# callmeray/PointMVSNet

Measured on AMD Instinct MI355X. Metric: depth-maps/sec (DTU 640x512, 3 src views, 2 flow iters), higher is better.
Workload: dtype f32

## Files before the change

### include/pointflow_hip.h

```cpp
#ifndef POINTFLOW_HIP_H_
#define POINTFLOW_HIP_H_

#include <stdint.h>

#ifdef __cplusplus
extern "C" {
#endif

#define PF_OK 0
#define PF_ERR_INVALID_ARG (-1)
#define PF_ERR_UNSUPPORTED (-2)

#define PF_STATUS_BAD_INDEX 1u

#define PF_MAX_VIEWS 8
#define PF_GEMM_TILE 64

#define PF_CAM_KREF_INV 0
#define PF_CAM_RREF_INV 9
#define PF_CAM_TREF 18
#define PF_CAM_MEAN 21
#define PF_CAM_STD 24
#define PF_CAM_VIEWS 27
#define PF_CAM_VIEW_STRIDE 21
// ... 112 lines not shown

int pf_edge_backward_coeffs_f32(const double* partials, int G, int T, int cbn, int C, int concat, int groups_per_stat,
                                int Ng, int k, float* c1, float* c2, float* dgamma, float* dbeta, int accumulate,
                                void* stream);

int64_t pf_knn_inverse_workspace(int G, int Ng, int k);
int pf_knn_inverse(const int64_t* idx, int k, int G, int Ng, uint32_t* order, uint32_t* start, void* workspace,
                   int64_t workspace_bytes, void* stream);

int pf_norm_blocks(int64_t S);
int pf_channel_stats_f32(const float* x, int64_t N, int64_t C, int64_t S, double* partials, void* stream);
int pf_channel_affine_f32(const float* x, float* y, const float* scale, const float* shift, int64_t N, int64_t C,
                          int64_t S, int samples_per_stat, int relu, void* stream);
int pf_channel_bn_apply_f32(const float* x, float* y, const double* partials, int T, int64_t N, int64_t C, int64_t S,
                            int samples_per_stat, double count, const float* gamma, const float* beta,
                            float* running_mean, float* running_var, float momentum, float eps, int relu,
                            const float* addend, void* stream);
int pf_channel_bn_apply2_f32(const float* x1, const double* partials1, int T1, const float* gamma1, const float* beta1,
                             float* running_mean1, float* running_var1, float momentum1, float eps1, const float* x2,
                             const double* partials2, int T2, const float* gamma2, const float* beta2,
                             float* running_mean2, float* running_var2, float momentum2, float eps2, float* y, int64_t N,
                             int64_t C, int64_t S, int samples_per_stat, double count, void* stream);
int pf_channel_bn_fused_f32(const float* x, float* y, int64_t N, int64_t C, int64_t S, int samples_per_stat,
                            const float* gamma, const float* beta, float* running_mean, float* running_var,
                            float momentum, float eps, int relu, float* scale, float* shift, int ld_affine,
                            void* stream);

int pf_conv3d_blocks(int64_t Cin, int64_t Cout, int64_t Di, int64_t Hi, int64_t Wi, int stride);
int pf_conv3d_k3_f32(const float* x, const float* wp, float* y, int64_t N, int64_t Cin, int64_t Cout, int64_t Di,
                     int64_t Hi, int64_t Wi, int stride, const float* in_scale, const float* in_shift,
                     const pf_bn_job* in_bn, int samples_per_stat, double* partials, void* stream);
int pf_conv3d_pair_blocks(int64_t Cin, int64_t Cout, int64_t D, int64_t H, int64_t W);
int pf_conv3d_k3_pair_f32(const float* x, const float* wp, float* y, int64_t N, int64_t Cin, int64_t Cout, int64_t D,
                          int64_t H, int64_t W, double* partials, void* stream);
int pf_conv3d_k3_few_f32(const float* x, const float* w, float* y, int64_t N, int64_t Cin, int64_t Cout, int64_t D,
                         int64_t H, int64_t W, void* stream);

int pf_deconv3d_blocks(int64_t D, int64_t H, int64_t W);
int pf_deconv3d_k3s2_f32(const float* xa, const float* xb, const float* w, float* y, int64_t N, int64_t Cin,
                         int64_t Cout, int64_t D, int64_t H, int64_t W, const float* in_scale, const float* in_shift,
                         const pf_bn_job* in_bn, int samples_per_stat, double* partials, void* stream);

int pf_conv3d_bottom_supported(int64_t Cin, int64_t Cout, int stride);
int pf_conv3d_bottom_blocks(int64_t Di, int64_t Hi, int64_t Wi, int stride);
int pf_conv3d_bottom_f32(const float* x, const float* wp, float* y, int64_t N, int64_t Cin, int64_t Cout, int64_t Di,
                         int64_t Hi, int64_t Wi, int stride, const float* in_scale, const float* in_shift,
                         const pf_bn_job* in_bn, int samples_per_stat, double* partials, void* stream);
int pf_deconv3d_bottom_supported(int64_t Cin, int64_t Cout);
int pf_deconv3d_bottom_blocks(int64_t Di, int64_t Hi, int64_t Wi);
int pf_deconv3d_bottom_f32(const float* x, const float* wp, float* y, int64_t N, int64_t Cin, int64_t Cout, int64_t Di,
                           int64_t Hi, int64_t Wi, const float* in_scale, const float* in_shift, const pf_bn_job* in_bn,
                           int samples_per_stat, double* partials, void* stream);

int pf_conv2d_wide_supported(int64_t Cin, int64_t Cout, int kernel_size, int stride);
int pf_conv2d_wide_blocks(int64_t Cout, int64_t Hi, int64_t Wi, int stride);
int pf_conv2d_wide_f32(const float* x, const float* wp, float* y, int64_t N, int64_t Cin, int64_t Cout, int64_t Hi,
                       int64_t Wi, int kernel_size, int stride, const float* in_scale, const float* in_shift,
                       const pf_bn_job* in_bn, int samples_per_stat, double* partials, int out_channel_last,
                       void* stream);
int pf_conv2d_wide_sets_f32(const float* x, int x_layout, const float* wp, int64_t wp_set_stride, int sets, float* y,
                            int64_t N, int64_t Cin, int64_t Cout, int64_t Hi, int64_t Wi, int kernel_size, int stride,
                            const float* in_scale, const float* in_shift, const pf_bn_job* in_bn, int samples_per_stat,
                            double* partials, int out_channel_last, void* stream);

int pf_flow_head_f32(const float* Z, int64_t ldz, const float* scale, const float* shift, int ld_affine,
                     const pf_bn_job* in_bn, const float* w_out, const float* depth_in, int dh, int dw,
                     const float* interval, int h, int w, int ratio, float* flow_prob, float* depth_out,
// ... 117 lines not shown
```

### pointmvsnet_amd/_lib.py

```python
import ctypes
import os

import torch

_HERE = os.path.dirname(os.path.abspath(__file__))
LIB_PATH = os.environ.get("PF_LIB_PATH") or os.path.join(_HERE, "libpointflow_hip.so")

_vp, _i, _i64, _f, _d = ctypes.c_void_p, ctypes.c_int, ctypes.c_int64, ctypes.c_float, ctypes.c_double



class BnJob(ctypes.Structure):
    _fields_ = [("partials", _vp), ("T", ctypes.c_int32), ("pcols", ctypes.c_int32), ("col0", ctypes.c_int32),
                ("C", ctypes.c_int32), ("count", _d), ("unbias_n", _d), ("gamma", _vp), ("beta", _vp),
                ("running_mean", _vp), ("running_var", _vp), ("momentum", _f), ("eps", _f),
                ("G", ctypes.c_int32), ("groups_per_stat", ctypes.c_int32), ("scale", _vp), ("shift", _vp),
                ("ld_affine", ctypes.c_int32), ("rows4", ctypes.c_int32)]


class WgradItem(ctypes.Structure):
    _fields_ = [("gr", _vp), ("x", _vp)] + [(n, _i64) for n in ("N", "Cg", "Cx", "Do", "Ho", "Wo", "Di", "Hi", "Wi")] + \
               [(n, ctypes.c_int32) for n in ("KD", "KH", "KW", "stride", "pd", "ph", "pw", "x_samples_per_stat")] + \
               [("x_scale", _vp), ("x_shift", _vp), ("workspace", _vp), ("workspace_bytes", _i64)] + \
               [(n, _i64) for n in ("rows_P", "ldg", "ldx", "x_rows_per_stat")]


PROTOTYPES = {
    "pf_version": ([], ctypes.c_char_p),
    "pf_error_string": ([_i], ctypes.c_char_p),
    "pf_device_info": ([ctypes.POINTER(_i), ctypes.POINTER(_i), ctypes.c_char_p, _i], _i),
    "pf_debug_timestamp": ([_vp, _vp], _i),
    "pf_check_status": ([ctypes.POINTER(ctypes.c_uint), _vp], _i),
    "pf_gather_knn_forward_f32": ([_vp, _vp, _vp, _i64, _i64, _i64, _i64, _vp], _i),
    "pf_gather_knn_forward_f64": ([_vp, _vp, _vp, _i64, _i64, _i64, _i64, _vp], _i),
    "pf_gather_knn_backward_f32": ([_vp, _vp, _vp, _i64, _i64, _i64, _i64, _vp, _vp, _vp], _i),
    "pf_gather_knn_backward_f64": ([_vp, _vp, _vp, _i64, _i64, _i64, _i64, _vp, _vp, _vp], _i),
    "pf_knn_lattice_f32": ([_vp, ctypes.POINTER(_i64), _i64, _i64, _i64, _i64, _i, _i, _vp, _vp, _vp], _i),
    "pf_fetch_forward_f32": ([_vp, _vp, _vp, _vp, _vp, _i64, _i64, _i64, _i64, _i64, _i64, _vp], _i),
    "pf_fetch_backward_f32": ([_vp, _vp, _vp, _vp, _vp, _i64, _i64, _i64, _i64, _i64, _i64, _vp], _i),
    "pf_fetch_variance_f32": ([_vp, _vp, _vp, _vp, _vp, _i64, _i64, _i64, _i64, _i64, _i64, _i, _vp], _i),
    "pf_frustum_variance_f32": ([_vp, _vp, _vp, _vp, _vp, _vp, _vp, _vp, _vp, _i64, _i64, _i64, _i64, _i64, _i64, _vp], _i),
    "pf_frustum_variance_cl_f32": ([_vp, _vp, _vp, _vp, _vp, _vp, _vp, _vp, _vp, _i64, _i64, _i64, _i64, _i64, _i64, _vp], _i),
    "pf_nchw_to_nhwc_f32": ([_vp, _vp, _i64, _i64, _i64, _vp], _i),
    "pf_resize_bilinear_f32": ([_vp, _vp, _i64, _i64, _i64, _i64, _i64, _vp], _i),
    "pf_flow_pyramid_f32": ([_vp, _i, _i, _i, _vp, _i, _i, _i, _vp, _i, _i, _i, _i, _i, _i, _vp, _vp, _vp,
                             ctypes.POINTER(_vp), ctypes.POINTER(_vp), _vp], _i),
    "pf_flow_features_f32": ([_vp, _vp, _vp, _i, _i, _i, _i, _i, _i, _vp, _i, _i, _vp, _vp, _i, _vp, _vp, _vp], _i),
    "pf_stat_blocks": ([_i, _i], _i),
    "pf_gemm_blocks": ([_i, _i], _i),
    "pf_pointwise_gemm_f32": ([_vp, _i, _i64, _vp, _vp, _i64, _i, _i, _i, _i, _i, _vp, _vp, ctypes.POINTER(BnJob), _i,
                               _vp, _vp], _i),
    "pf_conv3d_blocks": ([_i64, _i64, _i64, _i64, _i64, _i], _i),
    "pf_conv3d_k3_f32": ([_vp, _vp, _vp, _i64, _i64, _i64, _i64, _i64, _i64, _i, _vp, _vp, ctypes.POINTER(BnJob), _i,
                          _vp, _vp], _i),
    "pf_conv3d_pair_blocks": ([_i64, _i64, _i64, _i64, _i64], _i),
    "pf_conv3d_k3_pair_f32": ([_vp, _vp, _vp, _i64, _i64, _i64, _i64, _i64, _i64, _vp, _vp], _i),
    "pf_conv3d_k3_few_f32": ([_vp, _vp, _vp, _i64, _i64, _i64, _i64, _i64, _i64, _vp], _i),
    "pf_deconv3d_blocks": ([_i64, _i64, _i64], _i),
    "pf_deconv3d_k3s2_f32": ([_vp, _vp, _vp, _vp, _i64, _i64, _i64, _i64, _i64, _i64, _vp, _vp, ctypes.POINTER(BnJob), _i,
                              _vp, _vp], _i),
    "pf_conv3d_bottom_supported": ([_i64, _i64, _i], _i),
    "pf_conv3d_bottom_blocks": ([_i64, _i64, _i64, _i], _i),
    "pf_conv3d_bottom_f32": ([_vp, _vp, _vp, _i64, _i64, _i64, _i64, _i64, _i64, _i, _vp, _vp, ctypes.POINTER(BnJob), _i,
                              _vp, _vp], _i),
    "pf_deconv3d_bottom_supported": ([_i64, _i64], _i),
    "pf_deconv3d_bottom_blocks": ([_i64, _i64, _i64], _i),
    "pf_deconv3d_bottom_f32": ([_vp, _vp, _vp, _i64, _i64, _i64, _i64, _i64, _i64, _vp, _vp, ctypes.POINTER(BnJob), _i,
                                _vp, _vp], _i),
    "pf_conv2d_wide_supported": ([_i64, _i64, _i, _i], _i),
    "pf_conv2d_wide_blocks": ([_i64, _i64, _i64, _i], _i),
    "pf_conv2d_wide_f32": ([_vp, _vp, _vp, _i64, _i64, _i64, _i64, _i64, _i, _i, _vp, _vp, ctypes.POINTER(BnJob), _i,
                            _vp, _i, _vp], _i),
    "pf_conv2d_wide_sets_f32": ([_vp, _i, _vp, _i64, _i, _vp, _i64, _i64, _i64, _i64, _i64, _i, _i, _vp, _vp,
                                 ctypes.POINTER(BnJob), _i, _vp, _i, _vp], _i),
    "pf_norm_blocks": ([_i64], _i),
    "pf_channel_stats_f32": ([_vp, _i64, _i64, _i64, _vp, _vp], _i),
    "pf_channel_affine_f32": ([_vp, _vp, _vp, _vp, _i64, _i64, _i64, _i, _i, _vp], _i),
    "pf_channel_bn_apply_f32": ([_vp, _vp, _vp, _i, _i64, _i64, _i64, _i, _d, _vp, _vp, _vp, _vp, _f, _f, _i, _vp, _vp], _i),
    "pf_channel_bn_apply2_f32": ([_vp, _vp, _i, _vp, _vp, _vp, _vp, _f, _f, _vp, _vp, _i, _vp, _vp, _vp, _vp, _f, _f, _vp,
                                  _i64, _i64, _i64, _i, _d, _vp], _i),
    "pf_channel_bn_fused_f32": ([_vp, _vp, _i64, _i64, _i64, _i, _vp, _vp, _vp, _vp, _f, _f, _i, _vp, _vp, _i, _vp], _i),
    "pf_edge_stats_f32": ([_vp, _i64, _i, _vp, _i, _i, _i, _vp, _vp, _i, _i, _i, _vp], _i),
    "pf_edge_backward_reduce_f32": ([_vp, _i64, _i, _vp, _i, _i, _i, _vp, _i64, _vp, _vp, _vp, _vp, _i, _i, _i, _vp, _vp], _i),
    "pf_edge_backward_apply_f32": ([_vp, _i64, _i, _vp, _i, _i, _i, _vp, _i64, _vp, _vp, _vp, _vp, _vp, _vp, _i, _i, _i,
                                    _vp, _vp, _vp, _vp], _i),
    "pf_edge_backward_sums_f32": ([_vp, _i64, _i, _vp, _i, _i, _i, _vp, _i64, _vp, _vp, _vp, _vp, _i, _i, _i, _vp, _vp, _vp,
                                   _i64, _i, _vp], _i),
    "pf_edge_backward_finish_f32": ([_vp, _i64, _i, _i, _i, _i, _vp, _i64, _vp, _vp, _vp, _vp, _vp, _vp, _i, _i, _i,
                                     _vp, _vp, _vp, _i, _vp], _i),
# ... 189 lines not shown
```

### pointmvsnet_amd/csrc/conv3d_pair.hip

```cpp
#include <stdlib.h>

#include "pf_common.h"

namespace {

typedef float f32x4 __attribute__((ext_vector_type(4)));

struct PairGeom {
  int Cin, Cout, D, H, W;
  int tiles_d, tiles_h, tiles_w;
};

template <int TD>
struct PStage {
  static constexpr int ID = TD + 2;
  static constexpr int IH = 10;
  static constexpr int IW = 18;
  static constexpr int IWP = IW + 1;
  static constexpr int RAW = ID * IH * IWP;
  static constexpr int PLANE = RAW + ((16 - RAW % 32) + 32) % 32;
  static constexpr int ELEMS = ID * IH * IW;
  static constexpr int NXR = (ELEMS + 63) / 64;
};

constexpr int kTaps = 36;
constexpr int kWsz = kTaps * 4 * 16;

template <int TD>
constexpr size_t pair_lds_bytes() {
  using St = PStage<TD>;
  const size_t staging = sizeof(float) * (size_t)(2 * 4 * St::PLANE + 2 * kWsz);
  const size_t epilogue = sizeof(float) * (size_t)(4 * 16 * 17 + 1) + sizeof(double) * (size_t)(4 * 16 * 2);
  return staging > epilogue ? staging : epilogue;
}

template <int TD, int MINW>
__global__ __launch_bounds__(256, MINW) void conv3d_k3_pair_kernel(const float* __restrict__ x,
                                                                   const float* __restrict__ wp,
                                                                   float* __restrict__ y, PairGeom g,
                                                                   double* __restrict__ partials) {
  using St = PStage<TD>;
  constexpr int ID = St::ID, IH = St::IH, IW = St::IW, IWP = St::IWP, PLANE = St::PLANE;
  constexpr int ELEMS = St::ELEMS, NXR = St::NXR;
  constexpr int NWR = (kWsz + 255) / 256;
  constexpr int XS = 4 * PLANE;
  extern __shared__ __attribute__((aligned(16))) float lds[];
  float* xs0 = lds;
  float* ws0 = lds + 2 * XS;
  float* tile = lds;
  double* red = reinterpret_cast<double*>(tile + 4 * 16 * 17 + ((4 * 16 * 17) & 1));

  const int tid = threadIdx.x;
  const int wave = __builtin_amdgcn_readfirstlane(tid >> 6), lane = tid & 63;
  const int li = lane & 15, lk = lane >> 4;
  unsigned xb_, xn_;
  pf_xcd_xy<PF_XCD_CONV3D>(xb_, xn_);
  const int n = (int)xn_, bx = (int)xb_;
  const int plane_i = g.H * g.W, vol = plane_i * g.D;
  const float* xb = x + (int64_t)n * g.Cin * vol;
  float* yb = y + (int64_t)n * g.Cout * vol;
  const int cgroups = g.Cin >> 2;

  double ssum = 0.0, ssq = 0.0;

  const int total = g.tiles_d * g.tiles_h * g.tiles_w;
  for (int item = bx; item < total; item += gridDim.x) {
    const int tw = item % g.tiles_w;
    const int rest = item / g.tiles_w;
    const int th = rest % g.tiles_h;
    const int td = rest / g.tiles_h;
    const int od0 = td * TD, oh0 = th * 8, ow0 = tw * 16;
    const int id0 = od0 - 1, ih0 = oh0 - 1, iw0 = ow0 - 1;

    unsigned gofs[NXR];
    unsigned okmask = 0;
#pragma unroll
    for (int r = 0; r < NXR; ++r) {
      const int e = lane + 64 * r;
      const int row = e / IW, col = e - row * IW;
      const int dz = row / IH, hy = row - dz * IH;
      const int id = id0 + dz, ih = ih0 + hy, iw = iw0 + col;
      const bool ok = e < ELEMS && id >= 0 && id < g.D && ih >= 0 && ih < g.H && iw >= 0 && iw < g.W;
      gofs[r] = ok ? (unsigned)(id * plane_i + ih * g.W + iw) : 0u;
      okmask |= (ok ? 1u : 0u) << r;
    }

    float rx[NXR], rw[NWR];
    auto load_group = [&](int cg) {
      const float* src = xb + (int64_t)(cg * 4 + wave) * vol;
#pragma unroll
      for (int r = 0; r < NXR; ++r) rx[r] = src[gofs[r]];
      const float* wsrc = wp + (int64_t)cg * kWsz;
#pragma unroll
      for (int r = 0; r < NWR; ++r) {
        const int e = tid + 256 * r;
        rw[r] = (256 * (r + 1) <= kWsz || e < kWsz) ? wsrc[e] : 0.0f;
      }
    };
    auto store_group = [&](int buf) {
      float* xs = xs0 + buf * XS + wave * PLANE;
      float* ws = ws0 + buf * kWsz;
#pragma unroll
      for (int r = 0; r < NXR; ++r) {
        const int e = lane + 64 * r;
        if (64 * (r + 1) <= ELEMS || e < ELEMS) xs[e + e / IW] = ((okmask >> r) & 1u) ? rx[r] : 0.0f;
      }
#pragma unroll
      for (int r = 0; r < NWR; ++r) {
        const int e = tid + 256 * r;
        if (256 * (r + 1) <= kWsz || e < kWsz) ws[e] = rw[r];
      }
    };

    f32x4 acc[TD];
#pragma unroll
    for (int d = 0; d < TD; ++d) acc[d] = (f32x4){0.0f, 0.0f, 0.0f, 0.0f};

    __syncthreads();
    load_group(0);
    store_group(0);
    __syncthreads();
    for (int cg = 0; cg < cgroups; ++cg) {
      const int buf = cg & 1;
      if (cg + 1 < cgroups) load_group(cg + 1);
      const float* xs = xs0 + buf * XS + lk * PLANE + (2 * wave) * IWP + li;
      const float* ws = ws0 + buf * kWsz + lk * 16 + li;
#pragma unroll
      for (int kd = 0; kd < 3; ++kd) {
#pragma unroll
        for (int kh = 0; kh < 4; ++kh) {
#pragma unroll
          for (int kw = 0; kw < 3; ++kw) {
            const int tap = (kd * 4 + kh) * 3 + kw;
            const float b = ws[tap * 4 * 16];
#pragma unroll
            for (int d = 0; d < TD; ++d) {
              const float a = xs[((d + kd) * IH + kh) * IWP + kw];
              acc[d] = __builtin_amdgcn_mfma_f32_16x16x4f32(a, b, acc[d], 0, 0, 0);
            }
          }
        }
      }
      if (cg + 1 < cgroups) store_group(buf ^ 1);
      __syncthreads();
    }

    const int oh = oh0 + 2 * wave + (li >> 3);
    float* tl = tile + wave * 16 * 17;
#pragma unroll
    for (int d = 0; d < TD; ++d) {
      const int od = od0 + d;
      const bool row_ok = oh < g.H && od < g.D;
      float s = 0.0f, q = 0.0f;
#pragma unroll
      for (int r = 0; r < 4; ++r) {
        const int pos = lk * 4 + r;
        const float v = acc[d][r];
        tl[li * 17 + pos] = v;
        if (row_ok && ow0 + pos < g.W) {
          s += v;
          q += v * v;
        }
      }
      s += __shfl_xor(s, 8);
      q += __shfl_xor(q, 8);
      s += __shfl_xor(s, 16);
      q += __shfl_xor(q, 16);
      s += __shfl_xor(s, 32);
      q += __shfl_xor(q, 32);
      ssum += (double)s;
      ssq += (double)q;
      __builtin_amdgcn_wave_barrier();
      if (od < g.D) {
        for (int e = lane; e < 16 * 16; e += 64) {
          const int col = e >> 4, pos = e & 15;
          const int co = col & 7, ohh = oh0 + 2 * wave + (col >> 3);
          if (co < g.Cout && ohh < g.H && ow0 + pos < g.W)
            yb[(int64_t)co * vol + (int64_t)od * plane_i + (int64_t)ohh * g.W + ow0 + pos] = tl[col * 17 + pos];
        }
      }
      __builtin_amdgcn_wave_barrier();
    }
  }

  if (partials != nullptr) {
    if (lane < 8) {
      red[(wave * 16 + lane) * 2 + 0] = ssum;
      red[(wave * 16 + lane) * 2 + 1] = ssq;
    }
    __syncthreads();
    if (tid < g.Cout) {
      double s = 0.0, q = 0.0;
#pragma unroll
      for (int w = 0; w < 4; ++w) {
        s += red[(w * 16 + tid) * 2 + 0];
        q += red[(w * 16 + tid) * 2 + 1];
      }
      double* o = partials + (((int64_t)n * gridDim.x + bx) * g.Cout + tid) * 2;
      o[0] = s;
      o[1] = q;
    }
  }
}

#ifndef PF_PAIR_TD
#define PF_PAIR_TD 2
#endif
#ifndef PF_PAIR_MINW
#define PF_PAIR_MINW 3
#endif
constexpr int kPairTD = PF_PAIR_TD;

PairGeom make_pair_geom(int64_t Cin, int64_t Cout, int64_t D, int64_t H, int64_t W) {
  PairGeom g;
  g.Cin = (int)Cin;
  g.Cout = (int)Cout;
  g.D = (int)D;
  g.H = (int)H;
  g.W = (int)W;
  g.tiles_d = (g.D + kPairTD - 1) / kPairTD;
  g.tiles_h = (g.H + 7) / 8;
  g.tiles_w = (g.W + 15) / 16;
  return g;
}

int pair_blocks(const PairGeom& g) {
  const int64_t total = (int64_t)g.tiles_d * g.tiles_h * g.tiles_w;
#ifndef PF_CONV3D_CAP
#define PF_CONV3D_CAP 2048
#endif
  if (total <= PF_CONV3D_CAP) return (int)total;
  const int64_t per = (total + PF_CONV3D_CAP - 1) / PF_CONV3D_CAP;
  return (int)((total + per - 1) / per);
}

}

extern "C" {

int pf_conv3d_pair_blocks(int64_t Cin, int64_t Cout, int64_t D, int64_t H, int64_t W) {
  if (Cin <= 0 || Cout <= 0 || Cout > 8 || D <= 0 || H <= 0 || W <= 0) return 0;
  return pair_blocks(make_pair_geom(Cin, Cout, D, H, W));
}

int pf_conv3d_k3_pair_f32(const float* x, const float* wp, float* y, int64_t N, int64_t Cin, int64_t Cout, int64_t D,
                          int64_t H, int64_t W, double* partials, void* stream) {
  PF_REQUIRE(N >= 0 && Cin >= 4 && Cout >= 1 && D >= 1 && H >= 1 && W >= 1 && N <= 65535);
  if ((Cin % 4) != 0 || Cout > 8) return PF_ERR_UNSUPPORTED;
  PF_REQUIRE(Cin * D * H * W <= INT32_MAX);
  if (N == 0) return PF_OK;
  PF_REQUIRE(x && wp && y);
  const PairGeom g = make_pair_geom(Cin, Cout, D, H, W);
  constexpr size_t lds_bytes = pair_lds_bytes<kPairTD>();
  static_assert(lds_bytes <= 64 * 1024, "pair tile must fit the default dynamic LDS limit");
  dim3 grid((unsigned)pair_blocks(g), (unsigned)N);
  hipLaunchKernelGGL((conv3d_k3_pair_kernel<kPairTD, PF_PAIR_MINW>), grid, dim3(256), lds_bytes, (hipStream_t)stream, x, wp, y, g,
                     partials);
  return pf_launch_status();
}

}
```

### pointmvsnet_amd/networks.py

```python
import torch
import torch.nn as nn
import torch.nn.functional as F

from . import _lib
from . import pointflow
from .functions.gather_knn import gather_knn
from .nn.conv import *
from .nn.conv import Conv2d, Conv3d, Deconv3d


class _EdgeConvTrain(torch.autograd.Function):

    @staticmethod
    def forward(ctx, feature, knn_inds, w1, w2, gamma, beta, bn, concat):
        B, cin, N = feature.shape
        C = w1.shape[0]
        k = knn_inds.shape[2]
        width = (2 if concat else 1) * C
        x = feature.detach().float().contiguous()
        idx = knn_inds.contiguous()
        out = torch.empty((B * N, width), dtype=torch.float32, device=x.device)
        keep = {}
        with _lib.on_device(x.device):
            pointflow.edge_conv_fused(x, False, 0, cin, B, N, idx, w1, w2, bn, concat, out, width,
# ... 74 lines not shown
        if self.conv1.weight.shape[0] not in (32, 64) or knn_inds.shape[2] < 1:
            with torch.no_grad():
                return self._forward_autograd(feature, knn_inds)
        if feature.dtype == torch.float32:
            from . import graph
            return graph.module_forward(self, self._forward_fused, feature, knn_inds)
        return self._forward_fused(feature, knn_inds)


class EdgeConv(_EdgeConvBase):
    concat = True


class EdgeConvNoC(_EdgeConvBase):
    concat = False


def _deconv_block_ok(block):
    conv = getattr(block, "conv", None)
    return (type(conv) is nn.ConvTranspose3d and conv.kernel_size == (3, 3, 3) and conv.stride == (2, 2, 2)
            and conv.padding == (1, 1, 1) and conv.output_padding == (1, 1, 1) and conv.dilation == (1, 1, 1)
            and conv.groups == 1 and conv.bias is None)


def _deconv_fusable(block, x):
    return _deconv_block_ok(block) and x[0, 0].numel() >= 2048


def _conv3d_fusable(conv, x):
    return (type(conv) is nn.Conv3d and conv.kernel_size == (3, 3, 3) and conv.padding == (1, 1, 1)
            and conv.stride in ((1, 1, 1), (2, 2, 2)) and conv.dilation == (1, 1, 1) and conv.groups == 1
            and conv.bias is None and conv.in_channels % 4 == 0 and conv.out_channels <= 32
            and x[0, 0].numel() // (conv.stride[0] ** 3) >= 2048)


def _block_fused(block, x, samples_per_stat):
    skip = None
    if isinstance(x, tuple):
        x, skip = x
    if (skip is not None or hasattr(block, "bn")) and _deconv_fusable(block, x):
        training_bn = block.bn is not None and (block.bn.training or not block.bn.track_running_stats)
        y, partials = pointflow.deconv3d_k3s2(x.contiguous(), None if skip is None else skip.contiguous(),
                                              block.conv.weight, training_bn)
        if block.bn is not None:
            return pointflow.batch_norm_act_(y, block.bn, block.relu, samples_per_stat, partials=partials)
        return F.relu(y, inplace=True) if block.relu else y
    if not hasattr(block, "bn"):
        if (type(block) is nn.Conv3d and block.kernel_size == (3, 3, 3) and block.padding == (1, 1, 1)
                and block.stride == (1, 1, 1) and block.dilation == (1, 1, 1) and block.groups == 1
                and block.bias is None and block.out_channels <= 4 and block.in_channels * block.out_channels <= 256):
            return pointflow.conv3d_k3_few((x if skip is None else x + skip).contiguous(), block.weight)
        return block(x if skip is None else x + skip)
    if skip is not None:
        x = x + skip
    conv = block.conv
    training_bn = block.bn is not None and (block.bn.training or not block.bn.track_running_stats)
    if _conv3d_fusable(conv, x):
        y, partials = pointflow.conv3d_k3(x.contiguous(), conv.weight, conv.stride[0], training_bn)
        if block.bn is not None:
            return pointflow.batch_norm_act_(y, block.bn, block.relu, samples_per_stat, partials=partials)
        return F.relu(y, inplace=True) if block.relu else y
    pointflow.warn_library_fallback("VolumeConv layer", conv)
    y = block._crop(conv(x), x)
    if block.bn is not None:
        return pointflow.batch_norm_act_(y.contiguous(), block.bn, block.relu, samples_per_stat)
    return F.relu(y, inplace=True) if block.relu else y
# ... 120 lines not shown
    return pointflow.batch_norm_act_(y, bn, relu, samples_per_stat, partials=partials), None


class VolumeConv(nn.Module):

    def __init__(self, in_channels, base_channels):
        super(VolumeConv, self).__init__()
        b = base_channels
        self.in_channels = in_channels
        self.out_channels = 8 * b
        self.base_channels = b
        self.conv1_0 = Conv3d(in_channels, 2 * b, 3, stride=2, padding=1)
        self.conv2_0 = Conv3d(2 * b, 4 * b, 3, stride=2, padding=1)
        self.conv3_0 = Conv3d(4 * b, 8 * b, 3, stride=2, padding=1)
        self.conv0_1 = Conv3d(in_channels, b, 3, 1, padding=1)
        self.conv1_1 = Conv3d(2 * b, 2 * b, 3, 1, padding=1)
        self.conv2_1 = Conv3d(4 * b, 4 * b, 3, 1, padding=1)
        self.conv3_1 = Conv3d(8 * b, 8 * b, 3, 1, padding=1)
        self.conv4_0 = Deconv3d(8 * b, 4 * b, 3, 2, padding=1, output_padding=1)
        self.conv5_0 = Deconv3d(4 * b, 2 * b, 3, 2, padding=1, output_padding=1)
        self.conv6_0 = Deconv3d(2 * b, b, 3, 2, padding=1, output_padding=1)
        self.conv6_2 = nn.Conv3d(b, 1, 3, padding=1, bias=False)

    def _bottom_fusable(self):
        blocks = (self.conv3_0, self.conv3_1, self.conv4_0)
        return (all(b.bn is not None and b.relu for b in blocks)
                and pointflow.conv3d_bottom_supported(self.conv3_0.conv)
                and pointflow.conv3d_bottom_supported(self.conv3_1.conv)
                and pointflow.deconv3d_bottom_supported(self.conv4_0.conv))

    def forward_fused(self, x):
        B = x.shape[0]
        f = lambda blk, t: _block_fused(blk, t, B)
        blk0, blk6 = self.conv0_1, self.conv6_0
        train0 = blk0.bn is not None and blk0.relu and (blk0.bn.training or not blk0.bn.track_running_stats)
        if train0 and _conv3d_fusable(blk0.conv, x):
            full = pointflow.conv3d_k3(x.contiguous(), blk0.conv.weight, 1, True)
        else:
            full = f(blk0, x)
        pointflow.stamp("conv0_1_end")
        half = f(self.conv1_0, x)
        quarter = f(self.conv2_0, half)
        if self._bottom_fusable():
            b0, b1, b2 = self.conv3_0, self.conv3_1, self.conv4_0
            y0, p0 = pointflow.conv3d_bottom(quarter.contiguous(), b0.conv, None, B, True)
            y1, p1 = pointflow.conv3d_bottom(y0, b1.conv, pointflow.bn_affine_rows(y0, b0.bn, B, p0, lazy=True), B, True)
            pointflow.stamp("unet_encoder_end")
            y2, p2 = pointflow.deconv3d_bottom(y1, b2.conv, pointflow.bn_affine_rows(y1, b1.bn, B, p1, lazy=True), B, True)
            up = pointflow.batch_norm_act_(y2, b2.bn, b2.relu, B, partials=p2)
        else:
            eighth = f(self.conv3_1, f(self.conv3_0, quarter))
            pointflow.stamp("unet_encoder_end")
            up = f(self.conv4_0, eighth)
        pointflow.stamp("unet_bottom_end")
        half = f(self.conv1_1, half)
        quarter = f(self.conv2_1, quarter)
        up = f(self.conv5_0, (up, quarter))
        if (isinstance(full, tuple) and _deconv_fusable(blk6, up) and blk6.bn is not None and blk6.relu
                and (blk6.bn.training or not blk6.bn.track_running_stats)):
            y6, p6 = pointflow.deconv3d_k3s2(up.contiguous(), half.contiguous(), blk6.conv.weight, True)
            raw0, p0 = full
            return f(self.conv6_2, pointflow.batch_norm_act2_(raw0, blk0.bn, p0, y6, blk6.bn, p6, B))
        up = f(blk6, (up, half))
        if isinstance(full, tuple):
            raw, partials = full
            summed = pointflow.batch_norm_act_(raw, blk0.bn, blk0.relu, B, partials=partials, addend=up.contiguous())
        else:
            summed = up + full
        return f(self.conv6_2, summed)

    def forward(self, x):
        if pointflow.hip_inference(x, self):
            def run(v):
                y = self.forward_fused(v)
# ... 42 lines not shown
```

### pointmvsnet_amd/pointflow.py

```python
import contextlib
import ctypes

import torch

from . import _lib
from .utils.torch_utils import knn_lattice

_F32 = torch.float32


def hip_inference(x, module):
    if not (torch.is_tensor(x) and x.is_cuda and x.dtype == _F32):
        return False
    if not torch.is_grad_enabled():
        return True
    return not (x.requires_grad or any(p.requires_grad for p in module.parameters()))


_LIBRARY_WARNED = set()


def warn_library_fallback(what, conv):
    key = (what, type(conv).__name__, conv.in_channels, conv.out_channels, tuple(conv.kernel_size), tuple(conv.stride))
    if key in _LIBRARY_WARNED:
# ... 397 lines not shown
            torch._foreach_add_([t for t, _ in merged.values()], [n for _, n in merged.values()])


def eval_affine(bn, S, ld, ch0=0, C=None, out=None):
    C = bn.num_features - ch0 if C is None else C
    inv = torch.rsqrt(bn.running_var[ch0:ch0 + C] + bn.eps) * bn.weight.detach()[ch0:ch0 + C]
    sh = bn.bias.detach()[ch0:ch0 + C] - bn.running_mean[ch0:ch0 + C] * inv
    return inv, sh


def pack_conv3d_weight_pair(weight):
    def make():
        cout, cin = weight.shape[:2]
        w = weight.detach().to(_F32)
        wp = torch.zeros((cin // 4, 3, 4, 3, 4, 16), dtype=_F32, device=weight.device)
        src = w.permute(1, 2, 3, 4, 0).reshape(cin // 4, 4, 3, 3, 3, cout).permute(0, 2, 3, 4, 1, 5)
        for s_ in (0, 1):
            wp[:, :, s_:s_ + 3, :, :, 8 * s_:8 * s_ + cout] = src
        return wp.reshape(cin // 4, 36, 4, 16).contiguous()
    return _cached_pack(("c3p", id(weight)), (weight,), make)


def conv3d_k3(x, weight, stride, want_stats, in_affine=None, samples_per_stat=1):
    N, Cin, Di, Hi, Wi = x.shape
    Cout = weight.shape[0]
    if stride == 1 and Cout <= 8 and Cin % 4 == 0 and in_affine is None:
        wp = pack_conv3d_weight_pair(weight)
        y = torch.empty((N, Cout, Di, Hi, Wi), dtype=_F32, device=x.device)
        partials = None
        if want_stats:
            T = int(_lib.load().pf_conv3d_pair_blocks(Cin, Cout, Di, Hi, Wi))
            partials = torch.empty((N, T, Cout, 2), dtype=torch.float64, device=x.device)
        _lib.call("pf_conv3d_k3_pair_f32", _lib.ptr(x), _lib.ptr(wp), _lib.ptr(y), N, Cin, Cout, Di, Hi, Wi,
                  _lib.ptr(partials), _lib.stream(),
                  algo_bytes=4.0 * N * (Cin + Cout) * Di * Hi * Wi + 4.0 * 27 * Cin * Cout,
                  flops=2.0 * N * Di * Hi * Wi * 27 * Cin * Cout)
        return y, partials
    Do, Ho, Wo = (Di - 1) // stride + 1, (Hi - 1) // stride + 1, (Wi - 1) // stride + 1
    wp = pack_conv3d_weight(weight)
    y = torch.empty((N, Cout, Do, Ho, Wo), dtype=_F32, device=x.device)
    partials = None
    if want_stats:
        T = int(_lib.load().pf_conv3d_blocks(Cin, Cout, Di, Hi, Wi, int(stride)))
        partials = torch.empty((N, T, Cout, 2), dtype=torch.float64, device=x.device)
    sc, sh, in_bn = _split_affine(in_affine)
    _lib.call("pf_conv3d_k3_f32", _lib.ptr(x), _lib.ptr(wp), _lib.ptr(y), N, Cin, Cout, Di, Hi, Wi, int(stride),
              _lib.ptr(sc), _lib.ptr(sh), in_bn, int(samples_per_stat), _lib.ptr(partials), _lib.stream(),
              algo_bytes=4.0 * N * (Cin * Di * Hi * Wi + Cout * Do * Ho * Wo) + 4.0 * 27 * Cin * Cout,
              flops=2.0 * N * Do * Ho * Wo * 27 * Cin * Cout)
    return y, partials


def deconv3d_k3s2(xa, xb, weight, want_stats, in_affine=None, samples_per_stat=1):
    N, Cin, D, H, W = xa.shape
    Cout = weight.shape[1]
    w = weight.detach()
    if w.dtype != _F32 or not w.is_contiguous():
        w = w.to(_F32).contiguous()
    y = torch.empty((N, Cout, 2 * D, 2 * H, 2 * W), dtype=_F32, device=xa.device)
    partials = None
    if want_stats:
        T = int(_lib.load().pf_deconv3d_blocks(D, H, W))
        partials = torch.empty((N, T, Cout, 2), dtype=torch.float64, device=xa.device)
    vol = D * H * W
    sc, sh, in_bn = _split_affine(in_affine)
    _lib.call("pf_deconv3d_k3s2_f32", _lib.ptr(xa), _lib.ptr(xb), _lib.ptr(w), _lib.ptr(y), N, Cin, Cout, D, H, W,
              _lib.ptr(sc), _lib.ptr(sh), in_bn, int(samples_per_stat), _lib.ptr(partials), _lib.stream(),
              algo_bytes=4.0 * N * vol * (Cin * (2 if xb is not None else 1) + 8 * Cout) + 4.0 * 27 * Cin * Cout,
              flops=2.0 * N * vol * 27 * Cin * Cout)
    return y, partials


def conv2d_supported(conv):
    if type(conv) is not torch.nn.Conv2d or conv.bias is not None or conv.groups != 1 or conv.out_channels > 64:
        return False
    if conv.dilation != (1, 1):
        return False
    k3 = conv.kernel_size == (3, 3) and conv.stride == (1, 1) and conv.padding == (1, 1)
    k5 = conv.kernel_size == (5, 5) and conv.stride == (2, 2) and conv.padding == (2, 2)
    return k3 or k5


def conv2d_wide_supported(conv):
# ... 661 lines not shown
```

### pointmvsnet_amd/train_ops.py

```python
import torch

from . import _lib
from . import pointflow

import contextlib
import ctypes
import os

_F32 = torch.float32

_PACKS = None


@contextlib.contextmanager
def use_packs(packs):
    global _PACKS
    saved, _PACKS = _PACKS, packs
    try:
        if packs is None:
            yield None
        else:
            with packs.active():
                yield packs
    finally:
# ... 714 lines not shown
    for name in _VC_BLOCKS:
        blk = getattr(vc, name)
        ps += [blk.conv.weight, blk.bn.weight, blk.bn.bias]
    ps.append(vc.conv6_2.weight)
    return ps


class _VolumeTrain(torch.autograd.Function):
    @staticmethod
    def forward(ctx, cost, vc, *params):
        ctx.packs = _PACKS
        x0 = cost.detach().contiguous()
        assert x0.shape[0] == 1, "the fused VolumeConv training node is built for one scene per call"
        rec = {}

        def bn_act(name, y, partials, addend=None):
            blk = getattr(vc, name)
            S = y[0, 0].numel()
            if not TRAIN_LAZY_BN:
                rows = bn_train_rows(blk.bn, partials, 0, y.shape[1], float(S), 1, 1)
                z = channel_affine(y, rows, 1, True)
                return rows, (z if addend is None else z + addend)
            z = channel_bn_apply(y, blk.bn, partials, addend)
            return bn_rows(blk.bn, partials, y.shape[1], float(S), 1, 1, track=False, lazy=True).rows, z

        def conv(name, x, stride):
            blk = getattr(vc, name)
            y, p = pointflow.conv3d_k3(x, blk.conv.weight, stride, True)
            rows, z = bn_act(name, y, p)
            rec[name] = (x, y, rows)
            return z

        with torch.cuda.device(x0.device):
            z01 = conv("conv0_1", x0, 1)
            z10 = conv("conv1_0", x0, 2)
            z20 = conv("conv2_0", z10, 2)
            y30, p30 = pointflow.conv3d_bottom(z20, vc.conv3_0.conv, None, 1, True)
            r30, z30 = bn_act("conv3_0", y30, p30)
            rec["conv3_0"] = (z20, y30, r30)
            y31, p31 = pointflow.conv3d_bottom(z30, vc.conv3_1.conv, None, 1, True)
            r31, z31 = bn_act("conv3_1", y31, p31)
            rec["conv3_1"] = (z30, y31, r31)
            z11 = conv("conv1_1", z10, 1)
            z21 = conv("conv2_1", z20, 1)
            y40, p40 = pointflow.deconv3d_bottom(z31, vc.conv4_0.conv, None, 1, True)
            r40, s5 = bn_act("conv4_0", y40, p40, z21)
            rec["conv4_0"] = (z31, y40, r40)
            y50, p50 = pointflow.deconv3d_k3s2(s5, None, vc.conv5_0.conv.weight, True)
            r50, s6 = bn_act("conv5_0", y50, p50, z11)
            rec["conv5_0"] = (s5, y50, r50)
            y60, p60 = pointflow.deconv3d_k3s2(s6, None, vc.conv6_0.conv.weight, True)
            r60, s7 = bn_act("conv6_0", y60, p60, z01)
            rec["conv6_0"] = (s6, y60, r60)
            out = pointflow.conv3d_k3_few(s7, vc.conv6_2.weight)
            rec["conv6_2"] = (s7, None, None)
            pointflow.flush_counters()
        ctx.vc, ctx.rec = vc, rec
        return out

    @staticmethod
    @_with_packs
    def backward(ctx, gout):
        vc, rec = ctx.vc, ctx.rec
        grads = {}
        K3, P3 = (3, 3, 3), (1, 1, 1)

        def bnb(name, g):
            _, y, rows = rec[name]
# ... 467 lines not shown
```

Measured before the change: 1106.

## Fuse stride-2 conv1_0 into the conv0_1 pair kernel sharing input tiles

Result: no change. 1111, median of 6 (+0.5%).

```diff
diff --git a/include/pointflow_hip.h b/include/pointflow_hip.h
--- a/include/pointflow_hip.h
+++ b/include/pointflow_hip.h
@@ -168,7 +168,8 @@
                      const pf_bn_job* in_bn, int samples_per_stat, double* partials, void* stream);
 int pf_conv3d_pair_blocks(int64_t Cin, int64_t Cout, int64_t D, int64_t H, int64_t W);
 int pf_conv3d_k3_pair_f32(const float* x, const float* wp, float* y, int64_t N, int64_t Cin, int64_t Cout, int64_t D,
-                          int64_t H, int64_t W, double* partials, void* stream);
+                          int64_t H, int64_t W, double* partials, const float* wp2, float* y2, int64_t Cout2,
+                          double* partials2, void* stream);
 int pf_conv3d_k3_few_f32(const float* x, const float* w, float* y, int64_t N, int64_t Cin, int64_t Cout, int64_t D,
                          int64_t H, int64_t W, void* stream);
 
diff --git a/pointmvsnet_amd/_lib.py b/pointmvsnet_amd/_lib.py
--- a/pointmvsnet_amd/_lib.py
+++ b/pointmvsnet_amd/_lib.py
@@ -54,7 +54,7 @@
     "pf_conv3d_k3_f32": ([_vp, _vp, _vp, _i64, _i64, _i64, _i64, _i64, _i64, _i, _vp, _vp, ctypes.POINTER(BnJob), _i,
                           _vp, _vp], _i),
     "pf_conv3d_pair_blocks": ([_i64, _i64, _i64, _i64, _i64], _i),
-    "pf_conv3d_k3_pair_f32": ([_vp, _vp, _vp, _i64, _i64, _i64, _i64, _i64, _i64, _vp, _vp], _i),
+    "pf_conv3d_k3_pair_f32": ([_vp, _vp, _vp, _i64, _i64, _i64, _i64, _i64, _i64, _vp, _vp, _vp, _i64, _vp, _vp], _i),
     "pf_conv3d_k3_few_f32": ([_vp, _vp, _vp, _i64, _i64, _i64, _i64, _i64, _i64, _vp], _i),
     "pf_deconv3d_blocks": ([_i64, _i64, _i64], _i),
     "pf_deconv3d_k3s2_f32": ([_vp, _vp, _vp, _vp, _i64, _i64, _i64, _i64, _i64, _i64, _vp, _vp, ctypes.POINTER(BnJob), _i,
diff --git a/pointmvsnet_amd/csrc/conv3d_pair.hip b/pointmvsnet_amd/csrc/conv3d_pair.hip
--- a/pointmvsnet_amd/csrc/conv3d_pair.hip
+++ b/pointmvsnet_amd/csrc/conv3d_pair.hip
@@ -9,6 +9,7 @@
 struct PairGeom {
   int Cin, Cout, D, H, W;
   int tiles_d, tiles_h, tiles_w;
+  int Cout2, D2, H2, W2;
 };
 
 template <int TD>
@@ -25,30 +26,44 @@
 
 constexpr int kTaps = 36;
 constexpr int kWsz = kTaps * 4 * 16;
-
-template <int TD>
+constexpr int kW2sz = 27 * 4 * 16;
+
+template <int TD, bool S2>
+constexpr int pair_staging_floats() {
+  return 2 * 4 * PStage<TD>::PLANE + 2 * kWsz + (S2 ? kW2sz : 0);
+}
+
+template <int TD, bool S2>
 constexpr size_t pair_lds_bytes() {
-  using St = PStage<TD>;
-  const size_t staging = sizeof(float) * (size_t)(2 * 4 * St::PLANE + 2 * kWsz);
+  const size_t staging = sizeof(float) * (size_t)pair_staging_floats<TD, S2>();
   const size_t epilogue = sizeof(float) * (size_t)(4 * 16 * 17 + 1) + sizeof(double) * (size_t)(4 * 16 * 2);
-  return staging > epilogue ? staging : epilogue;
-}
-
-template <int TD, int MINW>
+  const size_t m = staging > epilogue ? staging : epilogue;
+  return S2 ? m + sizeof(double) * 2 * 4 * 16 * 2 : m;
+}
+
+template <int TD, int MINW, bool S2>
 __global__ __launch_bounds__(256, MINW) void conv3d_k3_pair_kernel(const float* __restrict__ x,
                                                                    const float* __restrict__ wp,
                                                                    float* __restrict__ y, PairGeom g,
-                                                                   double* __restrict__ partials) {
+                                                                   double* __restrict__ partials,
+                                                                   const float* __restrict__ wp2,
+                                                                   float* __restrict__ y2,
+                                                                   double* __restrict__ partials2) {
+  static_assert(!S2 || TD == 2, "the stride-2 layer takes one output plane per tile");
   using St = PStage<TD>;
   constexpr int ID = St::ID, IH = St::IH, IW = St::IW, IWP = St::IWP, PLANE = St::PLANE;
   constexpr int ELEMS = St::ELEMS, NXR = St::NXR;
   constexpr int NWR = (kWsz + 255) / 256;
+  constexpr int NW2 = S2 ? (kW2sz + 255) / 256 : 1;
   constexpr int XS = 4 * PLANE;
   extern __shared__ __attribute__((aligned(16))) float lds[];
   float* xs0 = lds;
   float* ws0 = lds + 2 * XS;
+  float* ws2 = ws0 + 2 * kWsz;
   float* tile = lds;
   double* red = reinterpret_cast<double*>(tile + 4 * 16 * 17 + ((4 * 16 * 17) & 1));
+  static_assert(pair_staging_floats<TD, S2>() % 2 == 0, "float64 statistics slots must be 8-byte aligned");
+  double* stat = reinterpret_cast<double*>(lds + pair_staging_floats<TD, S2>());
 
   const int tid = threadIdx.x;
   const int wave = __builtin_amdgcn_readfirstlane(tid >> 6), lane = tid & 63;
@@ -60,8 +75,11 @@
   const float* xb = x + (int64_t)n * g.Cin * vol;
   float* yb = y + (int64_t)n * g.Cout * vol;
   const int cgroups = g.Cin >> 2;
+  const int plane2 = g.H2 * g.W2;
+  float* y2b = S2 ? y2 + (int64_t)n * g.Cout2 * plane2 * g.D2 : nullptr;
 
   double ssum = 0.0, ssq = 0.0;
+  if constexpr (S2) stat[tid] = 0.0;
 
   const int total = g.tiles_d * g.tiles_h * g.tiles_w;
   for (int item = bx; item < total; item += gridDim.x) {
@@ -71,6 +89,8 @@
     const int td = rest / g.tiles_h;
     const int od0 = td * TD, oh0 = th * 8, ow0 = tw * 16;
     const int id0 = od0 - 1, ih0 = oh0 - 1, iw0 = ow0 - 1;
+    const int m2 = (wave - item) & 3;
+    const bool has2 = S2 && m2 < 2;
 
     unsigned gofs[NXR];
     unsigned okmask = 0;
@@ -85,7 +105,7 @@
       okmask |= (ok ? 1u : 0u) << r;
     }
 
-    float rx[NXR], rw[NWR];
+    float rx[NXR], rw[NWR], rw2[NW2];
     auto load_group = [&](int cg) {
       const float* src = xb + (int64_t)(cg * 4 + wave) * vol;
 #pragma unroll
@@ -95,6 +115,21 @@
       for (int r = 0; r < NWR; ++r) {
         const int e = tid + 256 * r;
         rw[r] = (256 * (r + 1) <= kWsz || e < kWsz) ? wsrc[e] : 0.0f;
+      }
+    };
+    auto load_w2 = [&](int cg) {
+      const float* w2src = wp2 + cg * kW2sz;
+#pragma unroll
+      for (int r = 0; r < NW2; ++r) {
+        const int e = tid + 256 * r;
+        rw2[r] = (256 * (r + 1) <= kW2sz || e < kW2sz) ? w2src[e] : 0.0f;
+      }
+    };
+    auto store_w2 = [&]() {
+#pragma unroll
+      for (int r = 0; r < NW2; ++r) {
+        const int e = tid + 256 * r;
+        if (256 * (r + 1) <= kW2sz || e < kW2sz) ws2[e] = rw2[r];
       }
     };
     auto store_group = [&](int buf) {
@@ -115,10 +150,15 @@
     f32x4 acc[TD];
 #pragma unroll
     for (int d = 0; d < TD; ++d) acc[d] = (f32x4){0.0f, 0.0f, 0.0f, 0.0f};
+    f32x4 acc2 = (f32x4){0.0f, 0.0f, 0.0f, 0.0f};
 
     __syncthreads();
     load_group(0);
     store_group(0);
+    if constexpr (S2) {
+      load_w2(0);
+      store_w2();
+    }
     __syncthreads();
     for (int cg = 0; cg < cgroups; ++cg) {
       const int buf = cg & 1;
@@ -141,8 +181,30 @@
           }
         }
       }
+      if (has2) {
+        const float* xs2 = xs0 + buf * XS + lk * PLANE + (2 * (2 * m2 + (li >> 3))) * IWP + 2 * (li & 7);
+        const float* wb2 = ws2 + lk * 16 + li;
+#pragma unroll
+        for (int kd = 0; kd < 3; ++kd) {
+#pragma unroll
+          for (int kh = 0; kh < 3; ++kh) {
+#pragma unroll
+            for (int kw = 0; kw < 3; ++kw) {
+              const int tap = (kd * 3 + kh) * 3 + kw;
+              acc2 = __builtin_amdgcn_mfma_f32_16x16x4f32(xs2[(kd * IH + kh) * IWP + kw], wb2[tap * 4 * 16], acc2, 0, 0, 0);
+            }
+          }
+        }
+      }
       if (cg + 1 < cgroups) store_group(buf ^ 1);
       __syncthreads();
+      if constexpr (S2) {
+        if (cg + 1 < cgroups) {
+          load_w2(cg + 1);
+          store_w2();
+          __syncthreads();
+        }
+      }
     }
 
     const int oh = oh0 + 2 * wave + (li >> 3);
@@ -168,8 +230,15 @@
       q += __shfl_xor(q, 16);
       s += __shfl_xor(s, 32);
       q += __shfl_xor(q, 32);
-      ssum += (double)s;
-      ssq += (double)q;
+      if constexpr (S2) {
+        if (lane < 8) {
+          stat[(wave * 16 + lane) * 2 + 0] += (double)s;
+          stat[(wave * 16 + lane) * 2 + 1] += (double)q;
+        }
+      } else {
+        ssum += (double)s;
+        ssq += (double)q;
+      }
       __builtin_amdgcn_wave_barrier();
       if (od < g.D) {
         for (int e = lane; e < 16 * 16; e += 64) {
@@ -181,10 +250,60 @@
       }
       __builtin_amdgcn_wave_barrier();
     }
+
+    if (has2) {
+      const int od2 = od0 >> 1;
+      double s = 0.0, q = 0.0;
+#pragma unroll
+      for (int r = 0; r < 4; ++r) {
+        const int row = lk * 4 + r;
+        const int oh2 = (oh0 >> 1) + 2 * m2 + (row >> 3), ow2 = (ow0 >> 1) + (row & 7);
+        const float v = acc2[r];
+        tl[li * 17 + row] = v;
+        if (od2 < g.D2 && oh2 < g.H2 && ow2 < g.W2) {
+          s += (double)v;
+          q += (double)v * (double)v;
+        }
+      }
+      s += __shfl_xor(s, 16);
+      q += __shfl_xor(q, 16);
+      s += __shfl_xor(s, 32);
+      q += __shfl_xor(q, 32);
+      if (lane < 16) {
+        stat[((4 + wave) * 16 + lane) * 2 + 0] += s;
+        stat[((4 + wave) * 16 + lane) * 2 + 1] += q;
+      }
+      __builtin_amdgcn_wave_barrier();
+      if (od2 < g.D2) {
+        for (int e = lane; e < 16 * 16; e += 64) {
+          const int co = e >> 4, row = e & 15;
+          const int oh2 = (oh0 >> 1) + 2 * m2 + (row >> 3), ow2 = (ow0 >> 1) + (row & 7);
+          if (co < g.Cout2 && oh2 < g.H2 && ow2 < g.W2)
+            y2b[(co * g.D2 + od2) * plane2 + oh2 * g.W2 + ow2] = tl[co * 17 + row];
+        }
+      }
+      __builtin_amdgcn_wave_barrier();
+    }
+  }
+
+  if constexpr (S2) {
+    __syncthreads();
+    red = stat;
+    if (partials2 != nullptr && tid < g.Cout2) {
+      double s = 0.0, q = 0.0;
+#pragma unroll
+      for (int w = 0; w < 4; ++w) {
+        s += stat[((4 + w) * 16 + tid) * 2 + 0];
+        q += stat[((4 + w) * 16 + tid) * 2 + 1];
+      }
+      double* o = partials2 + (((int64_t)n * gridDim.x + bx) * g.Cout2 + tid) * 2;
+      o[0] = s;
+      o[1] = q;
+    }
   }
 
   if (partials != nullptr) {
-    if (lane < 8) {
+    if (!S2 && lane < 8) {
       red[(wave * 16 + lane) * 2 + 0] = ssum;
       red[(wave * 16 + lane) * 2 + 1] = ssq;
     }
@@ -221,6 +340,10 @@
   g.tiles_d = (g.D + kPairTD - 1) / kPairTD;
   g.tiles_h = (g.H + 7) / 8;
   g.tiles_w = (g.W + 15) / 16;
+  g.Cout2 = 0;
+  g.D2 = (g.D + 1) / 2;
+  g.H2 = (g.H + 1) / 2;
+  g.W2 = (g.W + 1) / 2;
   return g;
 }
 
@@ -244,19 +367,37 @@
 }
 
 int pf_conv3d_k3_pair_f32(const float* x, const float* wp, float* y, int64_t N, int64_t Cin, int64_t Cout, int64_t D,
-                          int64_t H, int64_t W, double* partials, void* stream) {
+                          int64_t H, int64_t W, double* partials, const float* wp2, float* y2, int64_t Cout2,
+                          double* partials2, void* stream) {
   PF_REQUIRE(N >= 0 && Cin >= 4 && Cout >= 1 && D >= 1 && H >= 1 && W >= 1 && N <= 65535);
   if ((Cin % 4) != 0 || Cout > 8) return PF_ERR_UNSUPPORTED;
   PF_REQUIRE(Cin * D * H * W <= INT32_MAX);
+  if (wp2 != nullptr) {
+    PF_REQUIRE(Cout2 >= 1);
+    if (Cout2 > 16 || kPairTD != 2) return PF_ERR_UNSUPPORTED;
+  }
   if (N == 0) return PF_OK;
   PF_REQUIRE(x && wp && y);
-  const PairGeom g = make_pair_geom(Cin, Cout, D, H, W);
-  constexpr size_t lds_bytes = pair_lds_bytes<kPairTD>();
-  static_assert(lds_bytes <= 64 * 1024, "pair tile must fit the default dynamic LDS limit");
+  PairGeom g = make_pair_geom(Cin, Cout, D, H, W);
   dim3 grid((unsigned)pair_blocks(g), (unsigned)N);
-  hipLaunchKernelGGL((conv3d_k3_pair_kernel<kPairTD, PF_PAIR_MINW>), grid, dim3(256), lds_bytes, (hipStream_t)stream, x, wp, y, g,
-                     partials);
-  return pf_launch_status();
-}
-
-}
+  if (wp2 == nullptr) {
+    constexpr size_t lds_bytes = pair_lds_bytes<kPairTD, false>();
+    static_assert(lds_bytes <= 64 * 1024, "pair tile must fit the default dynamic LDS limit");
+    hipLaunchKernelGGL((conv3d_k3_pair_kernel<kPairTD, PF_PAIR_MINW, false>), grid, dim3(256), lds_bytes,
+                       (hipStream_t)stream, x, wp, y, g, partials, nullptr, nullptr, nullptr);
+    return pf_launch_status();
+  }
+  if constexpr (kPairTD == 2) {
+    PF_REQUIRE(y2 != nullptr);
+    g.Cout2 = (int)Cout2;
+    PF_REQUIRE((int64_t)g.Cout2 * g.D2 * g.H2 * g.W2 <= INT32_MAX);
+    constexpr size_t lds_bytes = pair_lds_bytes<kPairTD, true>();
+    static_assert(lds_bytes <= 160 * 1024 / 3, "the fused tile must leave room for three blocks per CU");
+    hipLaunchKernelGGL((conv3d_k3_pair_kernel<kPairTD, PF_PAIR_MINW, true>), grid, dim3(256), lds_bytes,
+                       (hipStream_t)stream, x, wp, y, g, partials, wp2, y2, partials2);
+    return pf_launch_status();
+  }
+  return PF_ERR_UNSUPPORTED;
+}
+
+}
diff --git a/pointmvsnet_amd/networks.py b/pointmvsnet_amd/networks.py
--- a/pointmvsnet_amd/networks.py
+++ b/pointmvsnet_amd/networks.py
@@ -130,6 +130,16 @@
             and conv.stride in ((1, 1, 1), (2, 2, 2)) and conv.dilation == (1, 1, 1) and conv.groups == 1
             and conv.bias is None and conv.in_channels % 4 == 0 and conv.out_channels <= 32
             and x[0, 0].numel() // (conv.stride[0] ** 3) >= 2048)
+
+
+def _pair_fusable(conv0, block1):
+    conv1 = getattr(block1, "conv", None)
+    bn1 = getattr(block1, "bn", None)
+    return (type(conv1) is nn.Conv3d and conv1.kernel_size == (3, 3, 3) and conv1.stride == (2, 2, 2)
+            and conv1.padding == (1, 1, 1) and conv1.dilation == (1, 1, 1) and conv1.groups == 1
+            and conv1.bias is None and conv0.stride == (1, 1, 1) and bn1 is not None
+            and (bn1.training or not bn1.track_running_stats)
+            and pointflow.conv3d_pair_fusable(conv0.weight, conv1.weight))
 
 
 def _block_fused(block, x, samples_per_stat):
@@ -316,14 +326,21 @@
     def forward_fused(self, x):
         B = x.shape[0]
         f = lambda blk, t: _block_fused(blk, t, B)
-        blk0, blk6 = self.conv0_1, self.conv6_0
+        blk0, blk6, blk10 = self.conv0_1, self.conv6_0, self.conv1_0
         train0 = blk0.bn is not None and blk0.relu and (blk0.bn.training or not blk0.bn.track_running_stats)
+        raw10 = None
         if train0 and _conv3d_fusable(blk0.conv, x):
-            full = pointflow.conv3d_k3(x.contiguous(), blk0.conv.weight, 1, True)
+            if _pair_fusable(blk0.conv, blk10):
+                full, raw10 = pointflow.conv3d_k3_pair_fused(x.contiguous(), blk0.conv.weight, blk10.conv.weight)
+            else:
+                full = pointflow.conv3d_k3(x.contiguous(), blk0.conv.weight, 1, True)
         else:
             full = f(blk0, x)
         pointflow.stamp("conv0_1_end")
-        half = f(self.conv1_0, x)
+        if raw10 is not None:
+            half = pointflow.batch_norm_act_(raw10[0], blk10.bn, blk10.relu, B, partials=raw10[1])
+        else:
+            half = f(blk10, x)
         quarter = f(self.conv2_0, half)
         if self._bottom_fusable():
             b0, b1, b2 = self.conv3_0, self.conv3_1, self.conv4_0
diff --git a/pointmvsnet_amd/pointflow.py b/pointmvsnet_amd/pointflow.py
--- a/pointmvsnet_amd/pointflow.py
+++ b/pointmvsnet_amd/pointflow.py
@@ -453,7 +453,7 @@
             T = int(_lib.load().pf_conv3d_pair_blocks(Cin, Cout, Di, Hi, Wi))
             partials = torch.empty((N, T, Cout, 2), dtype=torch.float64, device=x.device)
         _lib.call("pf_conv3d_k3_pair_f32", _lib.ptr(x), _lib.ptr(wp), _lib.ptr(y), N, Cin, Cout, Di, Hi, Wi,
-                  _lib.ptr(partials), _lib.stream(),
+                  _lib.ptr(partials), None, None, 0, None, _lib.stream(),
                   algo_bytes=4.0 * N * (Cin + Cout) * Di * Hi * Wi + 4.0 * 27 * Cin * Cout,
                   flops=2.0 * N * Di * Hi * Wi * 27 * Cin * Cout)
         return y, partials
@@ -470,6 +470,34 @@
               algo_bytes=4.0 * N * (Cin * Di * Hi * Wi + Cout * Do * Ho * Wo) + 4.0 * 27 * Cin * Cout,
               flops=2.0 * N * Do * Ho * Wo * 27 * Cin * Cout)
     return y, partials
+
+
+def conv3d_pair_fusable(weight, weight2):
+    return (weight.dim() == 5 and weight2.dim() == 5 and tuple(weight.shape[2:]) == (3, 3, 3)
+            and tuple(weight2.shape[2:]) == (3, 3, 3) and weight.shape[0] <= 8 and weight2.shape[0] <= 16
+            and weight.shape[1] == weight2.shape[1] and weight.shape[1] % 4 == 0)
+
+
+def conv3d_k3_pair_fused(x, weight, weight2):
+    N, Cin, D, H, W = x.shape
+    Cout, Cout2 = weight.shape[0], weight2.shape[0]
+    if not conv3d_pair_fusable(weight, weight2) or x.shape[1] != weight.shape[1]:
+        raise RuntimeError("conv3d_k3_pair_fused: unsupported layer pair %s / %s" % (tuple(weight.shape),
+                                                                                 tuple(weight2.shape)))
+    wp, wp2 = pack_conv3d_weight_pair(weight), pack_conv3d_weight(weight2)
+    D2, H2, W2 = (D + 1) // 2, (H + 1) // 2, (W + 1) // 2
+    y = torch.empty((N, Cout, D, H, W), dtype=_F32, device=x.device)
+    y2 = torch.empty((N, Cout2, D2, H2, W2), dtype=_F32, device=x.device)
+    T = int(_lib.load().pf_conv3d_pair_blocks(Cin, Cout, D, H, W))
+    partials = torch.empty((N, T, Cout, 2), dtype=torch.float64, device=x.device)
+    partials2 = torch.empty((N, T, Cout2, 2), dtype=torch.float64, device=x.device)
+    vol, vol2 = D * H * W, D2 * H2 * W2
+    _lib.call("pf_conv3d_k3_pair_f32", _lib.ptr(x), _lib.ptr(wp), _lib.ptr(y), N, Cin, Cout, D, H, W,
+              _lib.ptr(partials), _lib.ptr(wp2), _lib.ptr(y2), Cout2, _lib.ptr(partials2), _lib.stream(),
+              algo_bytes=(4.0 * N * (Cin + Cout) * vol + 4.0 * 27 * Cin * Cout)
+              + (4.0 * N * (Cin * vol + Cout2 * vol2) + 4.0 * 27 * Cin * Cout2),
+              flops=2.0 * N * vol * 27 * Cin * Cout + 2.0 * N * vol2 * 27 * Cin * Cout2)
+    return (y, partials), (y2, partials2)
 
 
 def deconv3d_k3s2(xa, xb, weight, want_stats, in_affine=None, samples_per_stat=1):
diff --git a/pointmvsnet_amd/train_ops.py b/pointmvsnet_amd/train_ops.py
--- a/pointmvsnet_amd/train_ops.py
+++ b/pointmvsnet_amd/train_ops.py
@@ -770,8 +770,16 @@
             return z
 
         with torch.cuda.device(x0.device):
-            z01 = conv("conv0_1", x0, 1)
-            z10 = conv("conv1_0", x0, 2)
+            w01, w10 = vc.conv0_1.conv.weight, vc.conv1_0.conv.weight
+            if pointflow.conv3d_pair_fusable(w01, w10):
+                (y01, p01), (y10, p10) = pointflow.conv3d_k3_pair_fused(x0, w01, w10)
+                rows01, z01 = bn_act("conv0_1", y01, p01)
+                rec["conv0_1"] = (x0, y01, rows01)
+                rows10, z10 = bn_act("conv1_0", y10, p10)
+                rec["conv1_0"] = (x0, y10, rows10)
+            else:
+                z01 = conv("conv0_1", x0, 1)
+                z10 = conv("conv1_0", x0, 2)
             z20 = conv("conv2_0", z10, 2)
             y30, p30 = pointflow.conv3d_bottom(z20, vc.conv3_0.conv, None, 1, True)
             r30, z30 = bn_act("conv3_0", y30, p30)
```
